# Jonas477/mixed-integer-optimal-control---algorithm-tools

Hardware: AMD Instinct MI355X
Metric: bellman_TRM! subproblems/sec (nt=65536, 4096 levels, budget=256) + HBM GB/s (higher is better)
Workload: dtype f64; 1 GPU; C4: nt=65536, 4096 levels (8x8x8x8 product), B=256, p=1, 1 subproblem(s) per GPU per step; parallelism=dp1 (independent subproblems; one GPU, no collective)

## Files before the change

include/mioc.h:

```cpp
#ifndef MIOC_H
#define MIOC_H

#include <stdint.h>

#ifdef __cplusplus
extern "C" {
#endif

#define MIOC_OK 0
#define MIOC_EINVAL -1
#define MIOC_EINEXACT -2
#define MIOC_ENOMEM -3
#define MIOC_EHIP -4
#define MIOC_EINFEASIBLE -5
#define MIOC_ESTATE -6
#define MIOC_ENONFINITE -7
#define MIOC_ECOMPILE -8

#define MIOC_P_INF 0
#define MIOC_P_ONE 1
#define MIOC_P_INTLUT 2
#define MIOC_P_TABLE 3

#define MIOC_OPT_ALGO 1
#define MIOC_ALGO_AUTO 0
#define MIOC_ALGO_GENERIC 1
#define MIOC_ALGO_PINF 2
#define MIOC_ALGO_PYRAMID 3
#define MIOC_ALGO_SEPARABLE 4
#define MIOC_ALGO_FUSED 5
#define MIOC_ALGO_FUSED_SEPARABLE 6
#define MIOC_OPT_TIMING 2
#define MIOC_OPT_PERSIST 3
#define MIOC_OPT_PRED_FMA 4
#define MIOC_OPT_SPIN_LIMIT 5
#define MIOC_OPT_SDT_BUFFERS 6
#define MIOC_OPT_FSEP_SEGMENTS 7
#define MIOC_OPT_PINF_WALK 8

typedef struct mioc_ctx mioc_ctx;

const char *mioc_version(void);

int32_t mioc_create(int32_t device, mioc_ctx **out);
int32_t mioc_destroy(mioc_ctx *ctx);
const char *mioc_last_error(const mioc_ctx *ctx);
int32_t mioc_set_option(mioc_ctx *ctx, int32_t option, int64_t value);

int32_t mioc_set_levels(mioc_ctx *ctx, int64_t M, const int64_t *counts, const int64_t *values, int64_t L,
                        const int32_t *tuples);

int32_t mioc_set_cost(mioc_ctx *ctx, int32_t p_kind, int64_t p_int, double beta, int64_t table_len,
                      const double *table);

int32_t mioc_bellman(mioc_ctx *ctx, const double *df, const double *u_old, int64_t nx, int64_t nt, int64_t B,
                     double dt);

int32_t mioc_backtrack(mioc_ctx *ctx, int64_t B_use, double *u_out, double *phi_star, uint8_t *switch_mask);

int32_t mioc_bellman_batch_device(mioc_ctx *ctx, int64_t K, const double *d_df, const double *d_u_old,
                                  int64_t nx, int64_t nt, int64_t B, double dt);
// ... 51 lines not shown
int32_t mioc_ode_program_eval_device(mioc_ctx *ctx, mioc_ode_program *prog, int64_t K, const double *d_x, int64_t nt,
                                     double T0, double T1, const double *state0, const double *params, double *d_J,
                                     double *d_df);

int32_t mioc_rand_start_device(mioc_ctx *ctx, int64_t K, int64_t nt, int64_t jumps, uint64_t seed, double *d_u_out);

int32_t mioc_heat_setup(mioc_ctx *ctx, int64_t N, int64_t nx, int64_t nt, double T0, double T1, double gamma,
                        const double *M_invA, const double *M_invF, const double *mass, const double *state0,
                        const double *yd);
int32_t mioc_heat_eval_device(mioc_ctx *ctx, int64_t K, const double *d_x, double *d_J, double *d_df);
int32_t mioc_heat_eval(mioc_ctx *ctx, int64_t K, const double *x, double *J, double *df);

int32_t mioc_conv_setup(mioc_ctx *ctx, int64_t nt, double T0, double T1, const double *kappa, const double *fvec);
int32_t mioc_conv_eval_device(mioc_ctx *ctx, int64_t K, const double *d_x, double *d_J, double *d_df);
int32_t mioc_conv_eval(mioc_ctx *ctx, int64_t K, const double *x, double *J, double *df);

void *mioc_stream(mioc_ctx *ctx);

int32_t mioc_kernel_stats(mioc_ctx *ctx, int32_t which, double *total_ms, int64_t *launches,
                          const char **name);
int32_t mioc_reset_stats(mioc_ctx *ctx);

int32_t mioc_last_algo(mioc_ctx *ctx);

int32_t mioc_diagnostics(mioc_ctx *ctx, int64_t *counters, int32_t n);

int32_t mioc_get_argmin_table(mioc_ctx *ctx, int64_t k, int64_t step, int32_t *U_out);

#ifdef __cplusplus
}
#endif
#endif
```

mixed-integer-optimal-control---algorithm-tools_amd/csrc/mioc_api.cpp:

```cpp
#include <hip/hip_runtime.h>

#include <algorithm>
#include <cmath>
#include <cstdio>
#include <cstring>
#include <new>
#include <string>
#include <thread>
#include <vector>

#include "mioc_internal.h"
#include "mioc_sdt_plan.h"

using namespace mioc;

namespace {

constexpr int kStats = 4;

int fail(mioc_ctx *ctx, int code, const std::string &msg) {
  if (ctx) ctx->err = msg;
  return code;
}

// ... 279 lines not shown
  const size_t stage_doubles = persist ? K * ks : 2 * K * s_stride;
  rc = ctx->d_stage.grow(ctx, stage_doubles * sizeof(double), "staging fronts");
  if (!rc) rc = ctx->d_U.grow(ctx, K * Y.uu_stride_k * sizeof(uint16_t), "argmin table U");
  if (rc) return rc;
  rc = ctx->d_perm.grow(ctx, K * nt * L * sizeof(uint32_t), "sphere orders");
  if (!rc) rc = ctx->d_same2.grow(ctx, K * nt * sizeof(int32_t), "sphere-order reuse flags");
  const bool seams = persist && sdt_seam_lists(ctx->pyr);
  if (!rc && seams) rc = ctx->d_strad.grow(ctx, K * nt * 8 * 32 * sizeof(uint16_t), "seam lists");
  if (rc) return rc;
  double *const stage = ctx->d_stage.get();
  uint16_t *const UU = (uint16_t *)ctx->d_U.get();
  uint32_t *const perm = ctx->d_perm.get();
  int32_t *const counters = ctx->d_counters.get();
  double *st[2] = {stage, stage + K * s_stride};
  double *term = persist ? stage + ((nt - 1) % plan.nbuf) * s_stride : st[(nt - 1) & 1];
  HIP_TRY(ctx, launch_pyr_order(ctx->stream, P, ctx->pyr, perm, ctx->d_same2.get(),
                                seams ? ctx->d_strad.get() : nullptr, counters));
  HIP_TRY(ctx, launch_pyr_terminal(ctx->stream, P, Lv, perm, term, ks));
  if (persist) {
    HIP_TRY(ctx, launch_sdt_prep(ctx->stream, P, Lv, ctx->pyr, perm, ctx->d_chain.get(), stage, ks,
                                 (size_t)plan.nbuf * s_stride, UU, Y.uu_stride_k));
    HIP_TRY(ctx, hipMemsetAsync(ctx->d_runflags.get(), 0, runflag_bytes, ctx->stream));
    ev_begin(ctx, 0, "k_sdt_run");
    HIP_TRY(ctx, launch_sdt_run(ctx->stream, P, Lv, ctx->pyr, perm, ctx->d_same2.get(), ctx->d_strad.get(), stage, ks,
                                plan.nbuf, UU, Y.uu_stride_k, counters, ctx->d_runflags.get(), plan.nwg,
                                ctx->spin_limit, run_lds));
    ev_end(ctx, 0, 1);
    Y.err_buf = &ctx->d_runflags, Y.err_off = nflag;
    return queue_timeout_read(ctx);
  }
  ev_begin(ctx, 0, sdt ? "k_sdt_step" : "k_pyr_step");
  for (int i = ctx->nt - 2; i >= 0; --i)
    HIP_TRY(ctx, (sdt ? launch_sdt_step : launch_pyr_step)(ctx->stream, P, Lv, ctx->pyr, i, perm, st[(i + 1) & 1],
                                                           st[i & 1], UU, s_stride, Y.uu_stride_k, counters));
  ev_end(ctx, 0, ctx->nt - 1);
  return MIOC_OK;
}

int fsep_segment_plan(const PyrGeom &G, size_t K, int B, int bmax, int want, int ncu, int cu_lds, int wg_lds,
                      FsepPlan *plan) {
  int S = want;
  if (S == 0) {
    S = 1;
    FsepPlan t;
    while (S < 8 && K * (size_t)(2 * S) <= (size_t)ncu && fsep2_plan(G, B, 2 * S, &t) && t.RS == t.W * (64 / t.lanes))
      S *= 2;
  }
  if (S > 1 && bmax > G.n[0] + G.n[1] - 2) S = 1;
  if (S < 1 || !fsep2_plan(G, B, S, plan)) return 0;
  if (S > 1 && K * (size_t)S <= (size_t)ncu) {
    const size_t half = std::min<size_t>((size_t)cu_lds / 2 + 2048, (size_t)wg_lds);
    plan->lds = std::max<size_t>(plan->lds, half);
  }
// ... 314 lines not shown
  return MIOC_OK;
}

const char *mioc_last_error(const mioc_ctx *ctx) { return ctx ? ctx->err.c_str() : "null context"; }

int32_t mioc_set_option(mioc_ctx *ctx, int32_t option, int64_t value) {
  if (!ctx) return MIOC_EINVAL;
  switch (option) {
    case MIOC_OPT_ALGO:
      if (value < MIOC_ALGO_AUTO || value > MIOC_ALGO_FUSED_SEPARABLE) return fail(ctx, MIOC_EINVAL, "unknown algorithm");
      ctx->opt_algo = value;
      return MIOC_OK;
    case MIOC_OPT_TIMING: ctx->timing = value != 0; return MIOC_OK;
    case MIOC_OPT_PERSIST: ctx->opt_persist = value != 0; return MIOC_OK;
    case MIOC_OPT_PRED_FMA: ctx->pred_fma = value != 0; return MIOC_OK;
    case MIOC_OPT_SPIN_LIMIT:
      if (value < 1 || value > (1ll << 30)) return fail(ctx, MIOC_EINVAL, "spin limit must be in [1, 2^30]");
      ctx->spin_limit = (unsigned)value;
      return MIOC_OK;
    case MIOC_OPT_SDT_BUFFERS:
      if (value < 4 || value > kSdtMaxBuffers) return fail(ctx, MIOC_EINVAL, "staging buffers must be in [4, 256]");
      ctx->opt_nb = (int)value;
      return MIOC_OK;
    case MIOC_OPT_PINF_WALK:
      if (value < -1 || value > 1) return fail(ctx, MIOC_EINVAL, "p=Inf walk option must be -1, 0 or 1");
      ctx->opt_pinf_walk = (int)value;
      return MIOC_OK;
    case MIOC_OPT_FSEP_SEGMENTS:
      if (value < -1 || value > 8) return fail(ctx, MIOC_EINVAL, "fused separable segments must be in [-1, 8]");
      ctx->opt_fsep_seg = (int)value;
      return MIOC_OK;
  }
  return fail(ctx, MIOC_EINVAL, "unknown option");
}

int32_t mioc_set_levels(mioc_ctx *ctx, int64_t M, const int64_t *counts, const int64_t *values, int64_t L,
                        const int32_t *tuples) {
  if (!ctx) return MIOC_EINVAL;
  MIOC_JOIN_BT(ctx);
  if (M < 1 || M > kMaxM) return fail(ctx, MIOC_EINVAL, "number of controls must be in [1, 8]");
  if (!counts || !values || !tuples) return fail(ctx, MIOC_EINVAL, "null level arrays");
  if (L < 1 || L > 65535) return fail(ctx, MIOC_EINVAL, "number of admissible tuples must be in [1, 65535]");
  std::vector<int64_t> off(M + 1, 0);
  int64_t Lgrid = 1;
  for (int64_t m = 0; m < M; ++m) {
    if (counts[m] < 1 || counts[m] > 4096) return fail(ctx, MIOC_EINVAL, "level count out of range");
// ... 510 lines not shown
  HIP_TRY(ctx, hipStreamSynchronize(ctx->stream));
  out[0] = ctx->h_trm_poll[0];
  out[1] = ctx->h_trm_poll[1];
  return MIOC_OK;
}

int32_t mioc_kernel_stats(mioc_ctx *ctx, int32_t which, double *total_ms, int64_t *launches, const char **name) {
  if (!ctx || which < 0 || which >= kStats) return MIOC_EINVAL;
  ev_collect(ctx);
  if (total_ms) *total_ms = ctx->stat_ms[which];
  if (launches) *launches = ctx->stat_launches[which];
  if (name) *name = ctx->stat_name[which];
  return MIOC_OK;
}

int32_t mioc_reset_stats(mioc_ctx *ctx) {
  if (!ctx) return MIOC_EINVAL;
  ev_collect(ctx);
  for (int w = 0; w < kStats; ++w) ctx->stat_ms[w] = 0.0, ctx->stat_launches[w] = 0;
  return MIOC_OK;
}

int32_t mioc_last_algo(mioc_ctx *ctx) { return ctx ? ctx->lay.algo : MIOC_EINVAL; }

int32_t mioc_diagnostics(mioc_ctx *ctx, int64_t *counters, int32_t n) {
  if (!ctx || !counters || n < 0) return MIOC_EINVAL;
  MIOC_JOIN_BT(ctx);
  HIP_TRY(ctx, hipSetDevice(ctx->device));
  int32_t c[8] = {0, 0, 0, 0, 0, 0, 0, 0}, f[4] = {0, 0, 0, 0};
  HIP_TRY(ctx, hipStreamSynchronize(ctx->stream));
  if (ctx->d_counters.get()) HIP_TRY(ctx, hipMemcpy(c, ctx->d_counters.get(), sizeof c, hipMemcpyDeviceToHost));
  HIP_TRY(ctx, hipMemcpy(f, ctx->d_flags.get(), sizeof f, hipMemcpyDeviceToHost));
  const int algo = ctx->lay.algo;
  const int64_t c6 = algo == MIOC_ALGO_SEPARABLE || algo == MIOC_ALGO_FUSED_SEPARABLE
                         ? ctx->n_persist_fallbacks
                         : algo == MIOC_ALGO_PINF ? ctx->n_persist_fallbacks + c[6] : c[6];
  int32_t fserial = -1;
  if (algo == MIOC_ALGO_PINF && ctx->last_pinf_fwalk && ctx->d_fneed.get())
    HIP_TRY(ctx, hipMemcpy(&fserial, ctx->d_fneed.get() + ctx->K, sizeof fserial, hipMemcpyDeviceToHost));
  const int64_t all[10] = {c[0], c[1], f[2], (int64_t)f[3] + c[3], c[4], c[5], c6, ctx->occupancy,
                           algo == MIOC_ALGO_FUSED_SEPARABLE ? ctx->last_fsep_seg : 0, fserial};
  for (int32_t q = 0; q < n && q < 10; ++q) counters[q] = all[q];
  return MIOC_OK;
}

int32_t mioc_get_argmin_table(mioc_ctx *ctx, int64_t k, int64_t step, int32_t *U_out) {
// ... 54 lines not shown
```

mixed-integer-optimal-control---algorithm-tools_amd/csrc/mioc_internal.h:

```cpp
#pragma once

#include <hip/hip_runtime.h>

#include <cstdint>
#include <cstdio>
#include <string>
#include <vector>

#include "../../include/mioc.h"

namespace mioc {

constexpr int kMaxM = 8;
constexpr int kRowTile = 64;

template <typename T>
struct DevBuf {
  DevBuf() = default;
  DevBuf(DevBuf &&o) noexcept : p(o.p), cap(o.cap) { o.p = nullptr, o.cap = 0; }
  DevBuf &operator=(DevBuf &&o) noexcept {
    if (this != &o) reset(), p = o.p, cap = o.cap, o.p = nullptr, o.cap = 0;
    return *this;
  }
  ~DevBuf() { reset(); }
// ... 135 lines not shown
hipError_t launch_pyr_order(hipStream_t s, const ProblemDev &P, const PyrGeom &G, uint32_t *perm,
                            int32_t *same2 = nullptr, uint16_t *strad = nullptr, int32_t *counters = nullptr);
hipError_t launch_pyr_terminal(hipStream_t s, const ProblemDev &P, const LevelsDev &Lv, const uint32_t *perm, double *S,
                               size_t s_stride);
hipError_t launch_pyr_step(hipStream_t s, const ProblemDev &P, const LevelsDev &Lv, const PyrGeom &G, int i,
                           const uint32_t *perm, const double *Sin, double *Sout, uint16_t *UU, size_t s_stride,
                           size_t uu_stride_k, int32_t *counters);
size_t pyr_lds_bytes(const PyrGeom &G);
bool sdt_supported(const PyrGeom &G);
bool sdt_seam_lists(const PyrGeom &G);
size_t sdt_lds_bytes(const PyrGeom &G);
constexpr int kSdtMaxBuffers = 256;
constexpr int kSdtDefaultBuffers = 256;
hipError_t launch_sdt_step(hipStream_t s, const ProblemDev &P, const LevelsDev &Lv, const PyrGeom &G, int i,
                           const uint32_t *perm, const double *Sin, double *Sout, uint16_t *UU, size_t s_stride,
                           size_t uu_stride_k, int32_t *counters);
hipError_t launch_sdt_prep(hipStream_t s, const ProblemDev &P, const LevelsDev &Lv, const PyrGeom &G,
                           const uint32_t *perm, double *V, double *S, size_t kstride, size_t r0off, uint16_t *UU,
                           size_t uu_stride_k);
hipError_t launch_sdt_run(hipStream_t s, const ProblemDev &P, const LevelsDev &Lv, const PyrGeom &G,
                          const uint32_t *perm, const int32_t *same2, const uint16_t *strad, double *S, size_t kstride,
                          int NB, uint16_t *UU,
                          size_t uu_stride_k, int32_t *counters, int32_t *flags, int nwg, unsigned spin_limit,
                          size_t lds);
int sdt_run_blocks_per_cu(const PyrGeom &G, size_t lds);
hipError_t launch_stage_argmin0(hipStream_t s, const ProblemDev &P, const LevelsDev &Lv, const uint32_t *perm,
                                const double *S0, size_t s_stride, int Bu, Start *start);
hipError_t launch_stage_walk(hipStream_t s, const ProblemDev &P, const LevelsDev &Lv, const uint16_t *UU,
                             size_t uu_stride_k, const Start *start, const int32_t *urank, int32_t *ranks,
                             int32_t *counters);

bool fused_supported(int L, int B, size_t *lds_out);
hipError_t launch_fused_run(hipStream_t s, const ProblemDev &P, const LevelsDev &Lv, double *front0,
                            size_t front_stride, uint8_t *U, size_t u_stride_k);
bool fsep_supported(const PyrGeom &G, int B, size_t *lds_out, int *threads_out);
int fused_blocks_per_cu(int algo_sep, const PyrGeom &G, int L, int B);
hipError_t launch_fsep_run(hipStream_t s, const ProblemDev &P, const LevelsDev &Lv, const PyrGeom &G, double *front0,
                           size_t front_stride, uint8_t *U, size_t u_stride_k, int32_t *counters);
struct FsepPlan {
  int S = 1, RS = 0, W = 0;
  int rows = 0, koff = 0;
  int stg = 0, slot_bytes = 0;
  int threads = 0;
  int lanes = 2;
  size_t lds = 0;
};
bool fsep2_plan(const PyrGeom &G, int B, int S, FsepPlan *out);
// ... 122 lines not shown
  int64_t tvw_len = 0;
  bool pred_fma = false;
  Buf<double> d_pred_own;
  bool trm_pending = false;
  const int32_t *Bvec = nullptr;
  Buf<double> d_ode_state;
  mioc::HeatState *heat = nullptr;
  mioc::ConvState *conv = nullptr;
  int64_t costlut_len = 0;

  bool have_dp = false;
  mioc::DpLayout lay;
  int K = 0, nt = 0, B = 0, RP = 0;
  double dt = 0.0;

  bool pyr_ok = false;
  bool grid_ok = false;
  mioc::PyrGeom pyr;
  Buf<double> d_stage;
  Buf<uint32_t> d_perm;
  Buf<int32_t> d_same2;
  Buf<uint16_t> d_strad;
  bool opt_persist = true;
  bool force_steps = false;
  int64_t n_persist_fallbacks = 0;
  Buf<int32_t> d_runflags;
  Buf<double> d_chain;
  unsigned spin_limit = 1u << 24;
  int opt_nb = mioc::kSdtDefaultBuffers;
  const int32_t *gate = nullptr;
  mioc::PinnedWord h_trm_poll;
  int opt_fsep_seg = 0;
  Buf<double> d_ring;
  Buf<int32_t> d_segflags;
  int last_fsep_seg = 0;
  mioc::PinnedWord h_run_err;
  bool run_pending = false;
  Buf<int32_t> d_counters;
  int64_t occupancy = 0;

  Buf<double> d_front;
  Buf<unsigned char> d_U;

  int pinf_BW = 0, pinf_BWP = 0, pinf_CH = 0, pinf_W = 0;
  Buf<uint8_t> d_ftab;
  Buf<int32_t> d_fseg, d_fneed;
// ... 49 lines not shown
```

mixed-integer-optimal-control---algorithm-tools_amd/csrc/mioc_sdt.hip:

```cpp
#include <hip/hip_runtime.h>

#include <cstdint>

#include "mioc_internal.h"
#include "mioc_sdt_common.h"

namespace mioc {

constexpr int SD_STRAD_N = 32;
template <int M>
__host__ __device__ constexpr bool sd_strad() {
  return M == 4;
}

#if defined(MIOC_STAMPS) && !defined(MIOC_STAMPS_TL)
__device__ unsigned long long g_sdt_stamps[4096][16];
#define SD_STAMP(k)                                                                          \
  do {                                                                                       \
    if (threadIdx.x == 0) sh.stamp[k] = __builtin_amdgcn_s_memtime();                         \
  } while (0)
#define SD_RSTAMP(k)                                                                         \
  do {                                                                                       \
    if (threadIdx.x == 0) sh.stamp[k] = __builtin_amdgcn_s_memrealtime();                     \
  } while (0)
// ... 725 lines not shown
    int bj = pj[0];
#pragma unroll
    for (int q = 1; q < NW; ++q)
      if (pv[q] < bv || (pv[q] == bv && (unsigned)pj[q] < (unsigned)bj)) {
        bv = pv[q];
        bj = pj[q];
      }
    const int l0 = (int)(e0h & 0xFFFFu);
    const bool fin = bj >= 0;
#pragma unroll
    for (int x = 0; x < 8; ++x) go[x] = INFINITY;
    if (tid == 0) {
      if (fin) go[0] = bv;
      outv[l0] = go[0];
      sh.cnt[1] += 1;
    }
    const bool mine = fin && tid == (l0 >> 3);
    const int sft = 16 * (l0 & 3);
    const unsigned long long cell = ~(0xFFFFull << sft) | ((unsigned long long)bj << sft);
    ut = make_ulonglong2(mine && !(l0 & 4) ? cell : ~0ull, mine && (l0 & 4) ? cell : ~0ull);
  } else {
    uint2 eo[4];
#pragma unroll
    for (int q = 0; q < 4; ++q) eo[q] = *reinterpret_cast<const uint2 *>(pout + sd_p2<M>(tid, q));
#pragma unroll
    for (int q = 0; q < 4; ++q) {
      go[2 * q] = outv[eo[q].x & 0xFFFFu];
      go[2 * q + 1] = outv[eo[q].y & 0xFFFFu];
    }
    ut = reinterpret_cast<const ulonglong2 *>(uu)[tid];
  }
  h.tail(empty, outv);
#pragma unroll
  for (int q = 0; q < 4; ++q)
    h.store16(Sout, sd_p2<M>(tid, q), __double_as_longlong(go[2 * q]), __double_as_longlong(go[2 * q + 1]));
  *reinterpret_cast<ulonglong2 *>(UU + 8 * tid) = ut;
  SD_STAMP(9);
  SD_RSTAMP(14);
  return empty ? 1 : 0;
}

template <int M, bool SC1>
__device__ __forceinline__ void sd_issue_loads(double (&v)[8], const uint32_t *pin, int cp, const double *Sin,
                                               int sbytes, const double *r0) {
  constexpr int L = 1 << (3 * M);
  const int tid = threadIdx.x;
#pragma unroll
// ... 153 lines not shown
    const double ov = sh.redv[q];
    const int oj = sh.redj[q];
    if (oj >= 0 && (bj < 0 || ov < bv || (ov == bv && oj < bj))) {
      bv = ov;
      bj = oj;
    }
  }
  __syncthreads();
  const bool wb = has0 && bj >= 0;
  if (has0 && tid == 0) atomicAdd(&counters[1], 1);
#pragma unroll
  for (int q = 0; q < 4; ++q) {
    const bool p0 = wb && sd_p2<M>(tid, q) == pm.pout_h;
    sd_store16<PERSIST>(SB, L * 8, sd_p2<M>(tid, q), p0 ? __double_as_longlong(bv) : 0x7FF0000000000000ull,
                        0x7FF0000000000000ull);
  }
  unsigned short ub[8];
#pragma unroll
  for (int x = 0; x < 8; ++x) ub[x] = wb && 8 * tid + x == r0 ? (unsigned short)bj : (unsigned short)0xFFFF;
  *reinterpret_cast<ulonglong2 *>(UB + 8 * tid) = make_ulonglong2(sd_pack4(ub), sd_pack4(ub + 4));
}

struct SdHooksNone {
  __device__ __forceinline__ void early() {}
  __device__ __forceinline__ void go() {}
  __device__ __forceinline__ void late_drain() {}
  __device__ __forceinline__ void publish() {}
  __device__ __forceinline__ void tail(bool, const double *) {}
  __device__ __forceinline__ void store16(double *Sout, int e, unsigned long long lo, unsigned long long hi) {
    sd_store16<false>(Sout, 0, e, lo, hi);
  }
};

size_t sdt_lds_bytes(const PyrGeom &G) { return G.M == 4 ? sd_lds_total<4>() : sd_lds_total<3>(); }

template <int M>
__device__ __forceinline__ void sd_perm_dma(const uint32_t *src, uint32_t *slot) {
  constexpr int L = 1 << (3 * M), T = L / 8, NW = T / 64;
  const int wave = threadIdx.x >> 6, lane = threadIdx.x & 63;
#pragma unroll
  for (int c = wave; c < L * 4 / 1024; c += NW)
    __builtin_amdgcn_global_load_lds(
        (const __attribute__((address_space(1))) void *)((const char *)src + c * 1024 + lane * 16),
        (__attribute__((address_space(3))) void *)((char *)slot + c * 1024), 16, 0, 0);
}

// ... 272 lines not shown
  for (int q = 0; q < 4; ++q) {
    const unsigned m = w.mask >> (3 * q);
    const double a0 = __hiloint2double((int)w.a[q].y, (int)w.a[q].x);
    const double a1 = __hiloint2double((int)w.a[q].w, (int)w.a[q].z);
    v[2 * q] = (m & 1) ? INFINITY : a0;
    if constexpr (sd_strad<M>()) {
      v[2 * q + 1] = (m & 4) ? __longlong_as_double(0x7FF8000000000000ll) : (m & 2) ? INFINITY : a1;
    } else {
      const double b1 = __hiloint2double((int)w.b[q].y, (int)w.b[q].x);
      v[2 * q + 1] = (m & 2) ? INFINITY : (m & 4) ? b1 : a1;
    }
  }
}


__device__ __forceinline__ int sd_flag_poll(const int32_t *p) {
  return __hip_atomic_load((const __attribute__((address_space(1))) int32_t *)p, __ATOMIC_RELAXED,
                           __HIP_MEMORY_SCOPE_AGENT);
}

template <int M>
struct SdPipe {
  static constexpr int L = 1 << (3 * M);
  int cp, i, ncp, ni;
  bool has_next;
  int lo, hi, B, nt, k, g0;
  int war;
  unsigned spin_limit, rowb, bufb, r0b;
  int32_t *dk, *lk, *err;
  const uint32_t *pk;
  uint32_t *slot;
  __amdgpu_buffer_rsrc_t rs;
  const char *dfuo0;
  unsigned dfuo_st;
  const uint16_t *sk;
  uint16_t *sslot;
  unsigned char *sds;
  unsigned ldsb;
  __device__ __forceinline__ unsigned lds_slot(int step) const {
    return ldsb + (unsigned)sd_slot_offset<M>() + (unsigned)(step & 1) * (unsigned)(L * sizeof(uint32_t));
  }
  __device__ __forceinline__ unsigned lds_sslot(int step) const {
    return ldsb + (unsigned)sd_strad_offset<M>() + (unsigned)(step & 1) * (unsigned)(8 * SD_STRAD_N * sizeof(uint16_t));
  }
  SdtShared<(1 << (3 * M - 3)) / 64> *sh;
  int pcp, pi;
// ... 188 lines not shown
      sdt_body<M, true>(P, Lv, G, k, cp, i, h.valid_next, ein, pslot(i + 1), pslot(i), nullptr,
                        uu_i + (unsigned)cp * (unsigned)L, sh, sds, h, df_all, uo_all, par, h.raw.mask, h.raw.srank);
      par ^= 1;
      SD_TL(6);
      stop = h.stop_seen;
    }
    bi1 = bi;
    bi = bi == 0 ? NB - 1 : bi - 1;
    unsigned rows = (unsigned)R;
    asm volatile("" : "+s"(rows));
    uu_i = reinterpret_cast<uint16_t *>(reinterpret_cast<char *>(uu_i) - rows * (unsigned)(L * sizeof(uint16_t)));
    ++h.war;
  }
  if (sd_tid() == 0) {
    if (sh.cnt[0]) atomicAdd(&counters[0], sh.cnt[0]);
    if (sh.cnt[1]) atomicAdd(&counters[1], sh.cnt[1]);
    if (sh.cnt[2]) atomicAdd(&counters[4], sh.cnt[2]);
    if (sh.cnt[3]) atomicAdd(&counters[5], sh.cnt[3]);
  }
  SD_FLUSH();
  SD_TL_FLUSH(h.g0);
}

bool sdt_seam_lists(const PyrGeom &G) { return G.M == 4 && sd_strad<4>(); }

bool sdt_supported(const PyrGeom &G) {
  if (G.M != 3 && G.M != 4) return false;
  for (int m = 0; m < G.M; ++m)
    if (G.n[m] != 8) return false;
  return true;
}

hipError_t launch_sdt_prep(hipStream_t s, const ProblemDev &P, const LevelsDev &Lv, const PyrGeom &G,
                           const uint32_t *perm, double *V, double *S, size_t kstride, size_t r0off, uint16_t *UU,
                           size_t uu_stride_k) {
  if (!sdt_supported(G)) return hipErrorInvalidValue;
  if (G.M == 4) {
    hipLaunchKernelGGL(k_sdt_chain<4>, dim3(P.K), dim3(256), 0, s, P, G, Lv.beta, perm, V);
    hipLaunchKernelGGL(k_sdt_row0<4>, dim3(P.nt, P.K), dim3(512), 0, s, P, Lv, G, perm, (const double *)V, S, kstride,
                       r0off, UU, uu_stride_k);
  } else {
    hipLaunchKernelGGL(k_sdt_chain<3>, dim3(P.K), dim3(256), 0, s, P, G, Lv.beta, perm, V);
    hipLaunchKernelGGL(k_sdt_row0<3>, dim3(P.nt, P.K), dim3(64), 0, s, P, Lv, G, perm, (const double *)V, S, kstride,
                       r0off, UU, uu_stride_k);
  }
  return hipGetLastError();
}

hipError_t launch_sdt_run(hipStream_t s, const ProblemDev &P, const LevelsDev &Lv, const PyrGeom &G,
                          const uint32_t *perm, const int32_t *same2, const uint16_t *strad, double *S, size_t kstride,
                          int NB, uint16_t *UU,
                          size_t uu_stride_k, int32_t *counters, int32_t *flags, int nwg, unsigned spin_limit,
                          size_t lds) {
  if (!sdt_supported(G)) return hipErrorInvalidValue;
  void *args[] = {(void *)&P,     (void *)&Lv,       (void *)&G,         (void *)&perm,
                  (void *)&S,     (void *)&kstride,  (void *)&NB,        (void *)&UU,
                  (void *)&uu_stride_k, (void *)&counters, (void *)&flags, (void *)&nwg, (void *)&spin_limit,
                  (void *)&P.df,  (void *)&P.uold, (void *)&same2, (void *)&strad};
  if (G.M == 4) return hipLaunchKernel((const void *)k_sdt_run<4>, dim3(nwg), dim3(512), args, lds, s);
  return hipLaunchKernel((const void *)k_sdt_run<3>, dim3(nwg), dim3(64), args, lds, s);
}

int sdt_run_blocks_per_cu(const PyrGeom &G, size_t lds) {
  int n = 0;
  hipError_t e = G.M == 4 ? hipOccupancyMaxActiveBlocksPerMultiprocessor(&n, k_sdt_run<4>, 512, lds)
                          : hipOccupancyMaxActiveBlocksPerMultiprocessor(&n, k_sdt_run<3>, 64, lds);
  return e == hipSuccess ? n : 0;
}

hipError_t launch_sdt_step(hipStream_t s, const ProblemDev &P, const LevelsDev &Lv, const PyrGeom &G, int i,
                           const uint32_t *perm, const double *Sin, double *Sout, uint16_t *UU, size_t s_stride,
                           size_t uu_stride_k, int32_t *counters) {
  if (!sdt_supported(G)) return hipErrorInvalidValue;
  const dim3 grid(P.B >= 1 ? P.B : 1, P.K);
  const size_t lds = sdt_lds_bytes(G);
  if (G.M == 4)
    hipLaunchKernelGGL(k_sdt_step<4>, grid, dim3(512), lds, s, P, Lv, G, i, perm, Sin, Sout, UU, s_stride,
                       uu_stride_k, counters);
  else
    hipLaunchKernelGGL(k_sdt_step<3>, grid, dim3(64), lds, s, P, Lv, G, i, perm, Sin, Sout, UU, s_stride,
                       uu_stride_k, counters);
// ... 21 lines not shown
```

mixed-integer-optimal-control---algorithm-tools_amd/csrc/mioc_sdt_plan.h:

```cpp
#pragma once

#include <algorithm>
#include <cstddef>

namespace mioc {

struct SdtPlan {
  bool persist = false;
  int nwg = 0;
  int nbuf = 2;
  size_t s_stride = 0;
  size_t kstride = 0;
};

inline SdtPlan sdt_stage_plan(size_t K, size_t nt, int B, size_t L, int M, int bmax, int opt_nb, bool opt_persist,
                              bool force_steps, int ncu, int blocks_per_cu) {
  SdtPlan p;
  p.s_stride = (size_t)(B + 1) * L;
  if (opt_persist && nt >= 2 && B >= 1 && p.s_stride * sizeof(double) < (1ull << 31) && bmax <= 7 * M &&
      !force_steps) {
    const size_t slots = (size_t)ncu * (size_t)std::max(std::min(blocks_per_cu, 1), 0);
    const size_t per_k = std::min<size_t>((size_t)B, K ? slots / K : 0);
    p.nwg = (int)(per_k * K);
    p.persist = per_k >= 1;
  }
  const int nb_min = 7 * M + 1;
  p.nbuf = p.persist ? std::max(opt_nb, nb_min) : 2;
  if (p.persist) {
    const size_t cap = (1ull << 32) / sizeof(double);
    const size_t fit = cap > nt * L ? (cap - nt * L - 1) / p.s_stride : 0;
    if ((size_t)p.nbuf > fit) p.nbuf = (int)fit;
    if (p.nbuf < nb_min) p.persist = false, p.nbuf = 2;
  }
  p.kstride = p.persist ? (size_t)p.nbuf * p.s_stride + nt * L : p.s_stride;
  if (p.persist && p.kstride * sizeof(double) >= (1ull << 32)) p.persist = false, p.kstride = p.s_stride;
  return p;
}

}
```

mixed-integer-optimal-control---algorithm-tools_amd/mioc/native.py:

```python
from __future__ import annotations

import atexit
import ctypes
import math
import os
import sys
import weakref

import numpy as np

from .iterators import LevelTable

_PKG_ROOT = os.path.dirname(os.path.dirname(os.path.abspath(__file__)))
LIB_PATH = os.path.join(_PKG_ROOT, "lib", "libmioc.so")

MIOC_OK = 0
MIOC_EINVAL = -1
MIOC_EINEXACT = -2
MIOC_ENOMEM = -3
MIOC_EHIP = -4
MIOC_EINFEASIBLE = -5
MIOC_ESTATE = -6
MIOC_ENONFINITE = -7
MIOC_ECOMPILE = -8

MIOC_P_INF, MIOC_P_ONE, MIOC_P_INTLUT, MIOC_P_TABLE = 0, 1, 2, 3
MIOC_OPT_ALGO, MIOC_OPT_TIMING, MIOC_OPT_PERSIST, MIOC_OPT_PRED_FMA = 1, 2, 3, 4
MIOC_OPT_SPIN_LIMIT, MIOC_OPT_SDT_BUFFERS, MIOC_OPT_FSEP_SEGMENTS, MIOC_OPT_PINF_WALK = 5, 6, 7, 8
MIOC_ALGO_AUTO, MIOC_ALGO_GENERIC, MIOC_ALGO_PINF, MIOC_ALGO_PYRAMID, MIOC_ALGO_SEPARABLE = 0, 1, 2, 3, 4
MIOC_ALGO_FUSED, MIOC_ALGO_FUSED_SEPARABLE = 5, 6
MIOC_ODE_FISHING, MIOC_ODE_DOUBLETANK, MIOC_ODE_VANDERPOL = 1, 2, 3
MIOC_ODE_INT_EULER, MIOC_ODE_INT_HEUN, MIOC_ODE_INT_RK4 = 0, 1, 2
MIOC_ODE_INT_BEULER, MIOC_ODE_INT_MIDPOINT = 16, 17
MIOC_ODE_NEWTON_MAX, MIOC_ODE_NEWTON_TOL = 12, 1e-10

EXPORTED = [
    "mioc_version", "mioc_create", "mioc_destroy", "mioc_last_error", "mioc_set_option", "mioc_set_levels",
    "mioc_set_cost", "mioc_bellman", "mioc_backtrack", "mioc_bellman_batch_device",
    "mioc_backtrack_batch_device", "mioc_synchronize", "mioc_stream", "mioc_kernel_stats",
    "mioc_reset_stats", "mioc_last_algo", "mioc_diagnostics", "mioc_get_argmin_table", "mioc_get_ranks_device",
    "mioc_pred", "mioc_pred_batch_device", "mioc_tv_device", "mioc_trm_decide_device", "mioc_batch_multi",
    "mioc_ode_eval_device", "mioc_rand_start_device", "mioc_backtrack_batch_budgets_device",
    "mioc_heat_setup", "mioc_heat_eval_device", "mioc_heat_eval",
    "mioc_conv_setup", "mioc_conv_eval_device", "mioc_conv_eval",
    "mioc_trm_state_bytes", "mioc_trm_attach", "mioc_trm_outer_begin_device", "mioc_trm_inner_end_device",
    "mioc_trm_poll",
    "mioc_ode_program_create", "mioc_ode_program_destroy", "mioc_ode_program_eval_device",
    "mioc_ode_program_create_ex",
]


class MiocNativeError(RuntimeError):
    def __init__(self, code, msg):
        super().__init__(f"mioc error {code}: {msg}")
        self.code = code


class InexactError(MiocNativeError):
    """Non-integral |ν - u_old| -- the reference's InexactError (HelpFunctions.jl:37,57)."""


_lib = None

# ... 9 lines not shown
        import torch
    except ImportError:
        pass
    lib = ctypes.CDLL(p)
    vp, i32, i64, dbl = ctypes.c_void_p, ctypes.c_int32, ctypes.c_int64, ctypes.c_double
    sig = {
        "mioc_version": (ctypes.c_char_p, []),
        "mioc_create": (i32, [i32, ctypes.POINTER(vp)]),
        "mioc_destroy": (i32, [vp]),
        "mioc_last_error": (ctypes.c_char_p, [vp]),
        "mioc_set_option": (i32, [vp, i32, i64]),
        "mioc_set_levels": (i32, [vp, i64, vp, vp, i64, vp]),
        "mioc_set_cost": (i32, [vp, i32, i64, dbl, i64, vp]),
        "mioc_bellman": (i32, [vp, vp, vp, i64, i64, i64, dbl]),
        "mioc_backtrack": (i32, [vp, i64, vp, ctypes.POINTER(dbl), vp]),
        "mioc_bellman_batch_device": (i32, [vp, i64, vp, vp, i64, i64, i64, dbl]),
        "mioc_backtrack_batch_device": (i32, [vp, i64, vp, vp, vp]),
        "mioc_synchronize": (i32, [vp]),
        "mioc_stream": (vp, [vp]),
        "mioc_kernel_stats": (i32, [vp, i32, ctypes.POINTER(dbl), ctypes.POINTER(i64),
                                    ctypes.POINTER(ctypes.c_char_p)]),
        "mioc_reset_stats": (i32, [vp]),
        "mioc_last_algo": (i32, [vp]),
        "mioc_diagnostics": (i32, [vp, vp, i32]),
        "mioc_get_argmin_table": (i32, [vp, i64, i64, vp]),
        "mioc_get_ranks_device": (i32, [vp, vp]),
        "mioc_pred": (i32, [vp, ctypes.POINTER(dbl), ctypes.POINTER(dbl), ctypes.POINTER(dbl),
                            ctypes.POINTER(dbl)]),
        "mioc_pred_batch_device": (i32, [vp, vp, vp, vp, vp]),
        "mioc_tv_device": (i32, [vp, i64, vp, i64, i64, vp]),
        "mioc_trm_decide_device": (i32, [vp, i64, vp, vp, vp, vp, vp, dbl, vp, vp]),
        "mioc_batch_multi": (i32, [vp, i32, i64, vp, vp, i64, i64, i64, dbl, i64, vp, vp, vp]),
        "mioc_ode_eval_device": (i32, [vp, i32, i64, vp, i64, i64, dbl, dbl, vp, i32, vp, vp]),
        "mioc_rand_start_device": (i32, [vp, i64, i64, i64, ctypes.c_uint64, vp]),
        "mioc_backtrack_batch_budgets_device": (i32, [vp, vp, vp, vp, vp]),
        "mioc_heat_setup": (i32, [vp, i64, i64, i64, dbl, dbl, dbl, vp, vp, vp, vp, vp]),
        "mioc_heat_eval_device": (i32, [vp, i64, vp, vp, vp]),
        "mioc_heat_eval": (i32, [vp, i64, vp, vp, vp]),
        "mioc_conv_setup": (i32, [vp, i64, dbl, dbl, vp, vp]),
        "mioc_conv_eval_device": (i32, [vp, i64, vp, vp, vp]),
        "mioc_conv_eval": (i32, [vp, i64, vp, vp, vp]),
        "mioc_trm_state_bytes": (i64, [i64]),
        "mioc_trm_attach": (i32, [vp, vp]),
        "mioc_trm_outer_begin_device": (i32, [vp, i64, vp, vp, dbl, i64, vp]),
        "mioc_trm_inner_end_device": (i32, [vp, i64, vp, dbl, i64, dbl, i64, vp, vp, vp, vp, vp, vp, vp, vp, i64, vp,
                                            vp, vp]),
# ... 373 lines not shown
        self._check(self.lib.mioc_rand_start_device(self.h, K, nt, int(jumps), ctypes.c_uint64(int(seed)),
                                                    ctypes.c_void_p(out.data_ptr())))

    def synchronize(self):
        self._check(self.lib.mioc_synchronize(self.h))

    def stream(self):
        return self.lib.mioc_stream(self.h)

    def kernel_stats(self, which=0):
        ms = ctypes.c_double(0)
        n = ctypes.c_int64(0)
        name = ctypes.c_char_p()
        self._check(self.lib.mioc_kernel_stats(self.h, int(which), ctypes.byref(ms), ctypes.byref(n),
                                               ctypes.byref(name)))
        return ms.value, n.value, (name.value or b"").decode()

    def reset_stats(self):
        self._check(self.lib.mioc_reset_stats(self.h))

    def last_algo(self):
        return self.lib.mioc_last_algo(self.h)

    def argmin_table(self, step, k=0):
        lg = int(np.prod(self.levels.counts))
        out = np.empty((lg, self.B + 1), dtype=np.int32)
        self._check(self.lib.mioc_get_argmin_table(self.h, int(k), int(step), _p(out)))
        return out.T

    def diagnostics(self):
        out = np.zeros(10, dtype=np.int64)
        self._check(self.lib.mioc_diagnostics(self.h, _p(out), 10))
        return out.tolist()


def batch_multi(ctxs, df, u_old, B, dt, B_use=None):
    df = np.ascontiguousarray(df, dtype=np.float64)
    u_old = np.ascontiguousarray(u_old, dtype=np.float64)
    if df.ndim != 3 or df.shape != u_old.shape:
        raise ValueError("df and u_old must have the same shape (K, nt, nx)")
    K, nt, nx = df.shape
    u = np.empty_like(df)
    phi = np.empty(K, dtype=np.float64)
    st = np.empty(K, dtype=np.int32)
    arr = (ctypes.c_void_p * len(ctxs))(*[c.h.value for c in ctxs])
    lib = ctxs[0].lib
# ... 47 lines not shown
```

Before: 2.482 subproblems/s.

## Add specialized one-row-per-workgroup persistent SDT kernel driver

Adds k_sdt_run1, a persistent SDT run kernel used when the planned workgroup count equals K*B, so each workgroup owns exactly one budget row for the whole backward sweep. Because each workgroup stays on one row, the per-step row-switch bookkeeping is dropped, the output-order indices are held in registers instead of being reloaded from memory, and the neighbour flag pointers are fixed once at startup. The path is on by default through a new option and is reported through a driver query. The cost is a second kernel variant to maintain and possible differences in register use or occupancy.

Result: faster. 2.554 subproblems/s, median of 6 (+2.9%).

```diff
diff --git a/include/mioc.h b/include/mioc.h
--- a/include/mioc.h
+++ b/include/mioc.h
@@ -37,6 +37,7 @@
 #define MIOC_OPT_SDT_BUFFERS 6
 #define MIOC_OPT_FSEP_SEGMENTS 7
 #define MIOC_OPT_PINF_WALK 8
+#define MIOC_OPT_SDT_ROW_OWNER 10
 
 typedef struct mioc_ctx mioc_ctx;
 
@@ -134,6 +135,7 @@
 int32_t mioc_reset_stats(mioc_ctx *ctx);
 
 int32_t mioc_last_algo(mioc_ctx *ctx);
+int32_t mioc_last_sdt_driver(mioc_ctx *ctx);
 
 int32_t mioc_diagnostics(mioc_ctx *ctx, int64_t *counters, int32_t n);
 
diff --git a/mixed-integer-optimal-control---algorithm-tools_amd/csrc/mioc_api.cpp b/mixed-integer-optimal-control---algorithm-tools_amd/csrc/mioc_api.cpp
--- a/mixed-integer-optimal-control---algorithm-tools_amd/csrc/mioc_api.cpp
+++ b/mixed-integer-optimal-control---algorithm-tools_amd/csrc/mioc_api.cpp
@@ -325,13 +325,16 @@
                                  (size_t)plan.nbuf * s_stride, UU, Y.uu_stride_k));
     HIP_TRY(ctx, hipMemsetAsync(ctx->d_runflags.get(), 0, runflag_bytes, ctx->stream));
     ev_begin(ctx, 0, "k_sdt_run");
+    const bool one_row = ctx->opt_row_owner && plan.one_row;
     HIP_TRY(ctx, launch_sdt_run(ctx->stream, P, Lv, ctx->pyr, perm, ctx->d_same2.get(), ctx->d_strad.get(), stage, ks,
                                 plan.nbuf, UU, Y.uu_stride_k, counters, ctx->d_runflags.get(), plan.nwg,
-                                ctx->spin_limit, run_lds));
+                                ctx->spin_limit, run_lds, one_row));
+    ctx->last_sdt_driver = one_row ? 2 : 1;
     ev_end(ctx, 0, 1);
     Y.err_buf = &ctx->d_runflags, Y.err_off = nflag;
     return queue_timeout_read(ctx);
   }
+  if (!ctx->force_steps) ctx->last_sdt_driver = 0;
   ev_begin(ctx, 0, sdt ? "k_sdt_step" : "k_pyr_step");
   for (int i = ctx->nt - 2; i >= 0; --i)
     HIP_TRY(ctx, (sdt ? launch_sdt_step : launch_pyr_step)(ctx->stream, P, Lv, ctx->pyr, i, perm, st[(i + 1) & 1],
@@ -692,6 +695,7 @@
       if (value < 4 || value > kSdtMaxBuffers) return fail(ctx, MIOC_EINVAL, "staging buffers must be in [4, 256]");
       ctx->opt_nb = (int)value;
       return MIOC_OK;
+    case MIOC_OPT_SDT_ROW_OWNER: ctx->opt_row_owner = value != 0; return MIOC_OK;
     case MIOC_OPT_PINF_WALK:
       if (value < -1 || value > 1) return fail(ctx, MIOC_EINVAL, "p=Inf walk option must be -1, 0 or 1");
       ctx->opt_pinf_walk = (int)value;
@@ -1248,6 +1252,8 @@
 }
 
 int32_t mioc_last_algo(mioc_ctx *ctx) { return ctx ? ctx->lay.algo : MIOC_EINVAL; }
+
+int32_t mioc_last_sdt_driver(mioc_ctx *ctx) { return ctx ? ctx->last_sdt_driver : MIOC_EINVAL; }
 
 int32_t mioc_diagnostics(mioc_ctx *ctx, int64_t *counters, int32_t n) {
   if (!ctx || !counters || n < 0) return MIOC_EINVAL;
diff --git a/mixed-integer-optimal-control---algorithm-tools_amd/csrc/mioc_internal.h b/mixed-integer-optimal-control---algorithm-tools_amd/csrc/mioc_internal.h
--- a/mixed-integer-optimal-control---algorithm-tools_amd/csrc/mioc_internal.h
+++ b/mixed-integer-optimal-control---algorithm-tools_amd/csrc/mioc_internal.h
@@ -181,7 +181,7 @@
                           const uint32_t *perm, const int32_t *same2, const uint16_t *strad, double *S, size_t kstride,
                           int NB, uint16_t *UU,
                           size_t uu_stride_k, int32_t *counters, int32_t *flags, int nwg, unsigned spin_limit,
-                          size_t lds);
+                          size_t lds, bool one_row);
 int sdt_run_blocks_per_cu(const PyrGeom &G, size_t lds);
 hipError_t launch_stage_argmin0(hipStream_t s, const ProblemDev &P, const LevelsDev &Lv, const uint32_t *perm,
                                 const double *S0, size_t s_stride, int Bu, Start *start);
@@ -350,6 +350,8 @@
   Buf<int32_t> d_same2;
   Buf<uint16_t> d_strad;
   bool opt_persist = true;
+  bool opt_row_owner = true;
+  int last_sdt_driver = 0;
   bool force_steps = false;
   int64_t n_persist_fallbacks = 0;
   Buf<int32_t> d_runflags;
diff --git a/mixed-integer-optimal-control---algorithm-tools_amd/csrc/mioc_sdt.hip b/mixed-integer-optimal-control---algorithm-tools_amd/csrc/mioc_sdt.hip
--- a/mixed-integer-optimal-control---algorithm-tools_amd/csrc/mioc_sdt.hip
+++ b/mixed-integer-optimal-control---algorithm-tools_amd/csrc/mioc_sdt.hip
@@ -771,7 +771,12 @@
   } else {
     uint2 eo[4];
 #pragma unroll
-    for (int q = 0; q < 4; ++q) eo[q] = *reinterpret_cast<const uint2 *>(pout + sd_p2<M>(tid, q));
+    for (int q = 0; q < 4; ++q) {
+      if constexpr (Hooks::kOutOrderRegs)
+        eo[q] = h.raw.e[q];
+      else
+        eo[q] = *reinterpret_cast<const uint2 *>(pout + sd_p2<M>(tid, q));
+    }
 #pragma unroll
     for (int q = 0; q < 4; ++q) {
       go[2 * q] = outv[eo[q].x & 0xFFFFu];
@@ -971,6 +976,7 @@
 }
 
 struct SdHooksNone {
+  static constexpr bool kOutOrderRegs = false;
   __device__ __forceinline__ void early() {}
   __device__ __forceinline__ void go() {}
   __device__ __forceinline__ void late_drain() {}
@@ -1289,6 +1295,7 @@
 template <int M>
 struct SdPipe {
   static constexpr int L = 1 << (3 * M);
+  static constexpr bool kOutOrderRegs = false;
   int cp, i, ncp, ni;
   bool has_next;
   int lo, hi, B, nt, k, g0;
@@ -1523,6 +1530,234 @@
   SD_TL_FLUSH(h.g0);
 }
 
+template <int M>
+struct SdPipe1 {
+  static constexpr int L = 1 << (3 * M);
+  static constexpr bool kOutOrderRegs = true;
+  int cp, i;
+  bool has_next;
+  int nt, k, g0;
+  unsigned spin_limit, rowb, r0b;
+  int32_t *lflag, *dflag, *err;
+  const uint32_t *pk;
+  uint32_t *slot;
+  __amdgpu_buffer_rsrc_t rs;
+  const char *dfuo0;
+  unsigned dfuo_st;
+  const uint16_t *sk;
+  uint16_t *sslot;
+  unsigned char *sds;
+  unsigned ldsb;
+  __device__ __forceinline__ unsigned lds_slot(int step) const {
+    return ldsb + (unsigned)sd_slot_offset<M>() + (unsigned)(step & 1) * (unsigned)(L * sizeof(uint32_t));
+  }
+  __device__ __forceinline__ unsigned lds_sslot(int step) const {
+    return ldsb + (unsigned)sd_strad_offset<M>() + (unsigned)(step & 1) * (unsigned)(8 * SD_STRAD_N * sizeof(uint16_t));
+  }
+  SdtShared<(1 << (3 * M - 3)) / 64> *sh;
+  int32_t *fp;
+  int need, val;
+  SdRaw raw;
+  SdNext nx;
+  const ProblemDev *Pp;
+  const PyrGeom *Gp;
+  unsigned valid_next;
+  unsigned nbo;
+  unsigned sob;
+  bool stop_seen;
+  double *reg;
+
+  __device__ __forceinline__ void early() {
+    SD_TL_AT(g0, i, nt, 1);
+    ++need;
+    if (!has_next && (sd_tid() & 63) < 32) need = INT32_MIN;
+    val = sd_flag_poll(fp);
+  }
+  __device__ __forceinline__ void go() {
+    SD_TL_AT(g0, i, nt, 2);
+    const int tid = sd_tid();
+    bool ready = __all(val >= need);
+    if (tid == 0) __hip_atomic_store(lflag, nt - 1 - i, __ATOMIC_RELAXED, __HIP_MEMORY_SCOPE_AGENT);
+    unsigned spins = 0;
+    while (!ready) {
+      if (sd_flag_poll(err) || ++spins > spin_limit) {
+        if ((tid & 63) == 0) {
+          __hip_atomic_store(err, 1, __ATOMIC_RELAXED, __HIP_MEMORY_SCOPE_AGENT);
+          sh->stop = 1;
+        }
+        break;
+      }
+      __builtin_amdgcn_s_sleep(1);
+      val = sd_flag_poll(fp);
+      ready = __all(val >= need);
+    }
+    SD_TL_AT(g0, i, nt, 3);
+    sd_read_next<M>(nx, slot + (i & 1) * L, sslot + (i & 1) * 8 * SD_STRAD_N);
+    if (has_next) {
+      const int ni = i - 1;
+      const int same = *(const volatile __attribute__((address_space(3))) int32_t *)(
+          sds + sd_dfuo_offset<M>() + (threadIdx.x >> 6) * sd_dfuo_stride<M>() + 16 * M);
+      sd_issue_pipe<M>(raw, rs, nx, cp, nbo, r0b + (unsigned)i * rowb, rowb);
+      if (!same) {
+        sd_perm_dma_asm<M>(pk + (size_t)ni * L, lds_slot(ni));
+        if constexpr (sd_strad<M>()) sd_strad_dma(sk + (size_t)ni * 8 * SD_STRAD_N, lds_sslot(ni));
+      }
+      sd_dfuo_dma<M>(dfuo0 + (size_t)((unsigned)ni * dfuo_st), ni >= 1, ldsb);
+    } else {
+#pragma unroll
+      for (int q = 0; q < 4; ++q) raw.e[q] = nx.e[q];
+    }
+    SD_TL_AT(g0, i, nt, 4);
+  }
+  __device__ __forceinline__ void late_drain() {
+#ifdef SD_TL_DRAIN
+    SD_TL_AT(g0, i, nt, 7);
+#endif
+    asm volatile("s_waitcnt vmcnt(0)" ::: "memory");
+    SD_TL_AT(g0, i, nt, 5);
+  }
+  __device__ __forceinline__ void publish() {
+    if (sd_tid() == 0 && i != nt - 2)
+      __hip_atomic_store(dflag, nt - 2 - i, __ATOMIC_RELAXED, __HIP_MEMORY_SCOPE_AGENT);
+    stop_seen = sh->stop != 0;
+  }
+  __device__ __forceinline__ void store16(double *, int e, unsigned long long lo, unsigned long long hi) {
+    sd_store16<true>(reg + sob / 8, L * 8, e, lo, hi);
+  }
+  __device__ __forceinline__ void tail(bool empty, const double *outv) {
+    if (!has_next) return;
+    double v[8];
+    sd_take<M>(v, raw);
+    if ((sd_tid() & 63) == 0 && (raw.e[0].x >> 16) == 0) v[0] = empty ? INFINITY : outv[raw.e[0].x & 0xFFFFu];
+    const double xs = __hiloint2double((int)raw.sv.y, (int)raw.sv.x);
+    valid_next = sdt_stats<M, true>(*Pp, *Gp, k, cp, i - 1, v, raw.e, *sh, sds, nullptr, nullptr, raw.srank, xs);
+  }
+};
+
+template <int M>
+__global__ __launch_bounds__(1 << (3 * M - 3), 2) void k_sdt_run1(ProblemDev P_arg, LevelsDev Lv_arg, PyrGeom G,
+                                                               const uint32_t *__restrict__ perm_all, double *S_all,
+                                                               size_t kstride, int NB, uint16_t *__restrict__ UU_all,
+                                                               size_t uu_stride_k, int32_t *__restrict__ counters,
+                                                               int32_t *flags, int nwg, unsigned spin_limit,
+                                                               const double *__restrict__ df_all,
+                                                               const double *__restrict__ uo_all,
+                                                               const int32_t *__restrict__ same2,
+                                                               const uint16_t *__restrict__ strad) {
+  constexpr int L = 1 << (3 * M);
+  extern __shared__ __attribute__((aligned(16))) unsigned char sds[];
+  __shared__ SdtShared<(1 << (3 * M - 3)) / 64> sh;
+  ProblemDev P = P_arg;
+  LevelsDev Lv = Lv_arg;
+  asm volatile("" : "+v"(P.dt), "+v"(Lv.beta), "+v"(Lv.inv_beta));
+  asm volatile("" : "+v"(counters), "+v"(spin_limit));
+  const int B = P.B, R = B + 1, nt = P.nt, tid = threadIdx.x;
+  const int FR = R * SDT_FLAG_STRIDE;
+  int32_t *done = flags, *loaded = flags + P.K * FR, *err = flags + 2 * P.K * FR;
+  const int k = (int)blockIdx.x / B, cp = 1 + (int)blockIdx.x - k * B;
+  if (k >= P.K) return;
+  (void)nwg;
+  uint32_t *slot = reinterpret_cast<uint32_t *>(sds + sd_slot_offset<M>());
+  auto pslot = [&](int step) { return slot + (step & 1) * L; };
+  double *reg = S_all + (size_t)k * kstride;
+  SdPipe1<M> h;
+  h.cp = cp, h.nt = nt, h.k = k, h.g0 = k * R + cp;
+  h.spin_limit = spin_limit, h.rowb = (unsigned)L * 8u;
+  const unsigned bufb = (unsigned)R * h.rowb;
+  h.r0b = (unsigned)NB * bufb;
+  asm volatile("" : "+v"(err));
+  h.err = err;
+  h.pk = perm_all + (size_t)k * nt * L, h.slot = slot;
+  h.rs = __builtin_amdgcn_make_buffer_rsrc(reg, 0, (int)(h.r0b + (unsigned)nt * h.rowb), 0x00020000);
+  h.dfuo0 = sd_dfuo_src<M>(df_all + (size_t)k * nt * M, uo_all + (size_t)k * nt * M, same2 + (size_t)k * nt - 1);
+  h.dfuo_st = sd_dfuo_step<M>();
+  h.sds = sds, h.ldsb = sd_lds_addr(sds), h.sh = &sh;
+  h.sk = strad ? strad + (size_t)k * nt * 8 * SD_STRAD_N : nullptr;
+  h.sslot = reinterpret_cast<uint16_t *>(sds + sd_strad_offset<M>());
+  {
+    int32_t *dk = done + (size_t)k * FR, *lk = loaded + (size_t)k * FR;
+    h.lflag = lk + cp * SDT_FLAG_STRIDE, h.dflag = dk + cp * SDT_FLAG_STRIDE;
+    const int lane = tid & 63, s = lane < 32 ? lane + 1 : lane - 31;
+    h.fp = h.lflag;
+    h.need = INT32_MIN;
+    if (lane < 32) {
+      if (s <= 7 * M && cp - s >= 1) h.fp = dk + (cp - s) * SDT_FLAG_STRIDE, h.need = 0;
+    } else {
+      if (s <= 7 * M && cp + s <= B) h.fp = lk + (cp + s) * SDT_FLAG_STRIDE, h.need = 1 - NB;
+    }
+    asm volatile("" : "+v"(h.lflag), "+v"(h.dflag));
+  }
+  asm volatile("" : "+v"(h.pk), "+v"(h.sk));
+  asm volatile("" : "+v"(h.r0b));
+  h.reg = reg;
+  if (tid == 0) {
+    sh.stop = 0;
+    sh.cnt[0] = sh.cnt[1] = sh.cnt[2] = sh.cnt[3] = 0;
+    sh.nlist[0] = sh.nlist[1] = sh.redo[0] = sh.redo[1] = 0;
+  }
+  sd_perm_dma_asm<M>(h.pk + (size_t)(nt - 1) * L, h.lds_slot(nt - 1));
+  sd_perm_dma_asm<M>(h.pk + (size_t)(nt - 2) * L, h.lds_slot(nt - 2));
+  if constexpr (sd_strad<M>()) {
+    sd_strad_dma(h.sk + (size_t)(nt - 1) * 8 * SD_STRAD_N, h.lds_sslot(nt - 1));
+    sd_strad_dma(h.sk + (size_t)(nt - 2) * 8 * SD_STRAD_N, h.lds_sslot(nt - 2));
+  }
+  sd_dfuo_dma<M>(h.dfuo0 + (size_t)((unsigned)(nt - 2) * h.dfuo_st), nt >= 3, h.ldsb);
+  asm volatile("s_waitcnt vmcnt(0)" ::: "memory");
+  sd_bar();
+  sd_read_next<M>(h.nx, pslot(nt - 1), h.sslot + ((nt - 1) & 1) * 8 * SD_STRAD_N);
+  sd_issue_pipe<M>(h.raw, h.rs, h.nx, cp, (unsigned)((nt - 1) % NB) * bufb, h.r0b + (unsigned)(nt - 1) * h.rowb,
+                   h.rowb);
+  __builtin_amdgcn_s_waitcnt(0x0F70);
+  h.Pp = &P, h.Gp = &G;
+  {
+    double v[8];
+    sd_take<M>(v, h.raw);
+    const double xs = __hiloint2double((int)h.raw.sv.y, (int)h.raw.sv.x);
+    h.valid_next = sdt_stats<M, true>(P, G, k, cp, nt - 2, v, h.raw.e, sh, sds, df_all, uo_all, h.raw.srank, xs);
+  }
+  const unsigned cprow = (unsigned)cp * h.rowb, wrapb = (unsigned)(NB - 1) * bufb;
+  h.nbo = (unsigned)((nt - 2) % NB) * bufb;
+  uint16_t *uu_i = UU_all + (size_t)k * uu_stride_k + (size_t)(nt - 2) * ((size_t)R * L) + (size_t)cp * L;
+  asm volatile("" : "+v"(uu_i));
+  int par = 0;
+  bool stop = false;
+  const int g = h.g0;
+  (void)g;
+  int i = nt - 2;
+#pragma nounroll
+  for (; i >= 0 && !stop; --i) {
+    h.i = i;
+    h.has_next = i >= 1;
+    h.sob = h.nbo + cprow;
+    SD_TL(0);
+    asm volatile("s_waitcnt vmcnt(5)" ::: "memory");
+#ifndef SD_TL_DRAIN
+    SD_TL(7);
+#endif
+    uint2 ein[4];
+#pragma unroll
+    for (int q = 0; q < 4; ++q) ein[q] = h.raw.e[q];
+    sdt_body<M, true>(P, Lv, G, k, cp, i, h.valid_next, ein, pslot(i + 1), pslot(i), nullptr, uu_i, sh, sds, h, df_all,
+                      uo_all, par, h.raw.mask, h.raw.srank);
+    par ^= 1;
+    SD_TL(6);
+    stop = h.stop_seen;
+    h.nbo = h.nbo == 0 ? wrapb : h.nbo - bufb;
+    unsigned rows = (unsigned)R;
+    asm volatile("" : "+s"(rows));
+    uu_i = reinterpret_cast<uint16_t *>(reinterpret_cast<char *>(uu_i) - rows * (unsigned)(L * sizeof(uint16_t)));
+  }
+  if (sd_tid() == 0) {
+    if (sh.cnt[0]) atomicAdd(&counters[0], sh.cnt[0]);
+    if (sh.cnt[1]) atomicAdd(&counters[1], sh.cnt[1]);
+    const int armed = cp < B ? max(nt - NB - 1 - i, 0) : 0;
+    if (armed) atomicAdd(&counters[4], armed);
+    if (sh.cnt[3]) atomicAdd(&counters[5], sh.cnt[3]);
+  }
+  SD_FLUSH();
+  SD_TL_FLUSH(h.g0);
+}
+
 bool sdt_seam_lists(const PyrGeom &G) { return G.M == 4 && sd_strad<4>(); }
 
 bool sdt_supported(const PyrGeom &G) {
@@ -1552,12 +1787,17 @@
                           const uint32_t *perm, const int32_t *same2, const uint16_t *strad, double *S, size_t kstride,
                           int NB, uint16_t *UU,
                           size_t uu_stride_k, int32_t *counters, int32_t *flags, int nwg, unsigned spin_limit,
-                          size_t lds) {
+                          size_t lds, bool one_row) {
   if (!sdt_supported(G)) return hipErrorInvalidValue;
+  if (one_row && nwg != P.K * P.B) return hipErrorInvalidValue;
   void *args[] = {(void *)&P,     (void *)&Lv,       (void *)&G,         (void *)&perm,
                   (void *)&S,     (void *)&kstride,  (void *)&NB,        (void *)&UU,
                   (void *)&uu_stride_k, (void *)&counters, (void *)&flags, (void *)&nwg, (void *)&spin_limit,
                   (void *)&P.df,  (void *)&P.uold, (void *)&same2, (void *)&strad};
+  if (one_row) {
+    if (G.M == 4) return hipLaunchKernel((const void *)k_sdt_run1<4>, dim3(nwg), dim3(512), args, lds, s);
+    return hipLaunchKernel((const void *)k_sdt_run1<3>, dim3(nwg), dim3(64), args, lds, s);
+  }
   if (G.M == 4) return hipLaunchKernel((const void *)k_sdt_run<4>, dim3(nwg), dim3(512), args, lds, s);
   return hipLaunchKernel((const void *)k_sdt_run<3>, dim3(nwg), dim3(64), args, lds, s);
 }
diff --git a/mixed-integer-optimal-control---algorithm-tools_amd/csrc/mioc_sdt_plan.h b/mixed-integer-optimal-control---algorithm-tools_amd/csrc/mioc_sdt_plan.h
--- a/mixed-integer-optimal-control---algorithm-tools_amd/csrc/mioc_sdt_plan.h
+++ b/mixed-integer-optimal-control---algorithm-tools_amd/csrc/mioc_sdt_plan.h
@@ -8,6 +8,7 @@
 struct SdtPlan {
   bool persist = false;
   int nwg = 0;
+  bool one_row = false;
   int nbuf = 2;
   size_t s_stride = 0;
   size_t kstride = 0;
@@ -34,6 +35,7 @@
   }
   p.kstride = p.persist ? (size_t)p.nbuf * p.s_stride + nt * L : p.s_stride;
   if (p.persist && p.kstride * sizeof(double) >= (1ull << 32)) p.persist = false, p.kstride = p.s_stride;
+  p.one_row = p.persist && (size_t)p.nwg == K * (size_t)B;
   return p;
 }
 
diff --git a/mixed-integer-optimal-control---algorithm-tools_amd/mioc/native.py b/mixed-integer-optimal-control---algorithm-tools_amd/mioc/native.py
--- a/mixed-integer-optimal-control---algorithm-tools_amd/mioc/native.py
+++ b/mixed-integer-optimal-control---algorithm-tools_amd/mioc/native.py
@@ -27,6 +27,7 @@
 MIOC_P_INF, MIOC_P_ONE, MIOC_P_INTLUT, MIOC_P_TABLE = 0, 1, 2, 3
 MIOC_OPT_ALGO, MIOC_OPT_TIMING, MIOC_OPT_PERSIST, MIOC_OPT_PRED_FMA = 1, 2, 3, 4
 MIOC_OPT_SPIN_LIMIT, MIOC_OPT_SDT_BUFFERS, MIOC_OPT_FSEP_SEGMENTS, MIOC_OPT_PINF_WALK = 5, 6, 7, 8
+MIOC_OPT_SDT_ROW_OWNER = 10
 MIOC_ALGO_AUTO, MIOC_ALGO_GENERIC, MIOC_ALGO_PINF, MIOC_ALGO_PYRAMID, MIOC_ALGO_SEPARABLE = 0, 1, 2, 3, 4
 MIOC_ALGO_FUSED, MIOC_ALGO_FUSED_SEPARABLE = 5, 6
 MIOC_ODE_FISHING, MIOC_ODE_DOUBLETANK, MIOC_ODE_VANDERPOL = 1, 2, 3
@@ -38,7 +39,8 @@
     "mioc_version", "mioc_create", "mioc_destroy", "mioc_last_error", "mioc_set_option", "mioc_set_levels",
     "mioc_set_cost", "mioc_bellman", "mioc_backtrack", "mioc_bellman_batch_device",
     "mioc_backtrack_batch_device", "mioc_synchronize", "mioc_stream", "mioc_kernel_stats",
-    "mioc_reset_stats", "mioc_last_algo", "mioc_diagnostics", "mioc_get_argmin_table", "mioc_get_ranks_device",
+    "mioc_reset_stats", "mioc_last_algo", "mioc_last_sdt_driver", "mioc_diagnostics", "mioc_get_argmin_table",
+    "mioc_get_ranks_device",
     "mioc_pred", "mioc_pred_batch_device", "mioc_tv_device", "mioc_trm_decide_device", "mioc_batch_multi",
     "mioc_ode_eval_device", "mioc_rand_start_device", "mioc_backtrack_batch_budgets_device",
     "mioc_heat_setup", "mioc_heat_eval_device", "mioc_heat_eval",
@@ -94,6 +96,7 @@
                                     ctypes.POINTER(ctypes.c_char_p)]),
         "mioc_reset_stats": (i32, [vp]),
         "mioc_last_algo": (i32, [vp]),
+        "mioc_last_sdt_driver": (i32, [vp]),
         "mioc_diagnostics": (i32, [vp, vp, i32]),
         "mioc_get_argmin_table": (i32, [vp, i64, i64, vp]),
         "mioc_get_ranks_device": (i32, [vp, vp]),
@@ -513,6 +516,9 @@
     def last_algo(self):
         return self.lib.mioc_last_algo(self.h)
 
+    def last_sdt_driver(self):
+        return self.lib.mioc_last_sdt_driver(self.h)
+
     def argmin_table(self, step, k=0):
         lg = int(np.prod(self.levels.counts))
         out = np.empty((lg, self.B + 1), dtype=np.int32)
```
